# drnatebrown/col-bwt

Hardware: AMD Instinct MI355X
Metric: query bases/s (higher is better)
Workload: dtype int64

## Files before the change

### col-bwt_amd/__init__.py

```python
import ctypes as C
import os

import numpy as np

_HERE = os.path.dirname(os.path.abspath(__file__))
LIB_PATH = os.path.join(_HERE, "libcolbwt.so")
HEADER_PATH = os.path.join(os.path.dirname(_HERE), "include", "colbwt.h")

EXPORTS = (
    "colbwt_version", "colbwt_last_error", "colbwt_index_open", "colbwt_index_open_memory",
    "colbwt_index_open_layout", "colbwt_index_open_memory_layout",
    "colbwt_index_open_devices", "colbwt_index_open_memory_devices",
    "colbwt_index_close", "colbwt_index_info", "colbwt_query_batch", "colbwt_query_batch_u32",
    "colbwt_query_device", "colbwt_query_device_ordered", "colbwt_query_file", "colbwt_query_file_binary",
    "colbwt_binary_to_text", "colbwt_synth_index_bytes", "colbwt_synth_index", "colbwt_synth_index_thr", "colbwt_pml_pack_device", "colbwt_read_end_mask_device", "colbwt_pml_unpack_device",
    "colbwt_index_cid_dictionary", "colbwt_cid_code_bits", "colbwt_cid_pack_device", "colbwt_cid_unpack_device",
    "colbwt_synth_reads_device", "colbwt_build_col_pml", "colbwt_build_col_pml_arrays",
    "colbwt_col_split", "colbwt_col_split_arrays", "colbwt_col_split_error",
    "colbwt_rlbwt_build_text", "colbwt_rlbwt_build_files", "colbwt_rlbwt_get", "colbwt_rlbwt_free", "colbwt_rlbwt_error",
    "colbwt_count_batch", "colbwt_count_device", "colbwt_count_file",
    "colbwt_index_attach_locate", "colbwt_index_attach_locate_memory", "colbwt_locate_docs", "colbwt_locate_batch",
    "colbwt_locate_device", "colbwt_locate_file",
    "colbwt_rlbwt_build_text_locate", "colbwt_rlbwt_build_files_locate", "colbwt_rlbwt_write_locate",
    "colbwt_seeds_reduce_device", "colbwt_seeds_batch", "colbwt_seeds_file",
)

SEED_NONE = 0xFFFFFFFF
SEED_SUMMARY = np.dtype([(k, np.uint32) for k in ("n_seeds", "max_len", "cov", "resets", "n_col", "col_cov", "asc", "desc")])
LOCATE_NONE = (1 << 64) - 1


class ColbwtError(RuntimeError):
    def __init__(self, code, msg):
        super().__init__(f"colbwt error {code}: {msg}")
        self.code = code


class Info(C.Structure):
    _fields_ = [("bwt_r", C.c_uint64), ("n", C.c_uint64), ("r", C.c_uint64), ("sigma", C.c_uint32),
                ("device", C.c_uint32), ("device_bytes", C.c_uint64), ("layout", C.c_uint32),
                ("layout_shape", C.c_uint32), ("table_rows", C.c_uint64), ("n_devices", C.c_uint32),
                ("reserved_", C.c_uint32)]


class Stats(C.Structure):
    _fields_ = [("n_reads", C.c_uint64), ("n_bases", C.c_uint64), ("h2d_ms", C.c_double),
                ("kernel_ms", C.c_double), ("d2h_ms", C.c_double), ("algorithmic_bytes", C.c_uint64)]

    def as_dict(self):
        return {k: getattr(self, k) for k, _ in self._fields_}


_lib = None


def lib():
    global _lib
    if _lib is not None:
        return _lib
    if not os.path.exists(LIB_PATH):
        raise ColbwtError(-100, f"{LIB_PATH} not built: run __graft_entry__.build() "
                                "(the query path has no CPU fallback)")
    try:
        import torch
    except ImportError:
# ... 77 lines not shown
        else:
            _check(lib().colbwt_index_open_layout(os.fsencode(prefix_or_file), None, int(device), int(layout),
                                                  C.byref(h)))
        return cls(h)

    @classmethod
    def from_bytes(cls, image, device=0, layout=0, devices=None):
        arr = np.ascontiguousarray(np.frombuffer(image, dtype=np.uint8))
        h = C.c_void_p()
        if devices is not None:
            dv = (C.c_int * len(devices))(*[int(d) for d in devices])
            _check(lib().colbwt_index_open_memory_devices(arr.ctypes.data, arr.size, None, dv, len(devices), int(layout),
                                                          C.byref(h)))
        else:
            _check(lib().colbwt_index_open_memory_layout(arr.ctypes.data, arr.size, None, int(device), int(layout),
                                                         C.byref(h)))
        return cls(h)

    def info(self):
        out = Info()
        _check(lib().colbwt_index_info(self._h, C.byref(out)))
        return out

    def query_pml(self, pattern):
        p = np.frombuffer(bytes(pattern), dtype=np.uint8)
        off = np.array([0, p.size], dtype=np.uint64)
        pml, cid, _ = self.query_batch(p, off, wide=p.size > 65535)
        return pml.astype(np.uint64), cid.astype(np.uint64)

    def query_batch(self, bases, read_off, wide=False):
        bases = np.ascontiguousarray(bases, dtype=np.uint8)
        read_off = np.ascontiguousarray(read_off, dtype=np.uint64)
        n_reads = read_off.size - 1
        total = int(read_off[-1]) if n_reads >= 0 and read_off.size else 0
        pml = np.zeros(total, np.uint32 if wide else np.uint16)
        cid = np.zeros(total, np.uint8)
        st = Stats()
        fn = lib().colbwt_query_batch_u32 if wide else lib().colbwt_query_batch
        _check(fn(self._h, bases.ctypes.data, read_off.ctypes.data, max(n_reads, 0),
                  pml.ctypes.data, cid.ctypes.data, C.byref(st)))
        return pml, cid, st

    def query_device(self, d_bases, d_read_off, n_reads, n_bases, d_pml, d_cid, pml_bytes=2,
                     stream=0, timed=False, d_order=None):
        st = Stats()
        _check(lib().colbwt_query_device_ordered(self._h, d_bases, d_read_off, n_reads, n_bases, d_pml,
# ... 329 lines not shown
```

### col-bwt_amd/csrc/capi.hip

```cpp
#include <fcntl.h>
#include <hip/hip_runtime.h>
#include <stdlib.h>
#include <string.h>
#include <sys/mman.h>
#include <sys/stat.h>
#include <unistd.h>

#include <algorithm>
#include <atomic>
#include <chrono>
#include <condition_variable>
#include <deque>
#include <mutex>
#include <string>
#include <thread>
#include <vector>

#include "../../include/colbwt.h"
#include "bin_writer.h"
#include "count_query.h"
#include "fasta_parallel.h"
#include "fastx_reader.h"
#include "index.h"
#include "locate_query.h"
// ... 859 lines not shown
int colbwt_index_open_devices(const char *prefix_or_file, const colbwt_widths *widths, const int *devices, int n_devices,
                              int layout, colbwt_index **out) {
    if (!prefix_or_file || !out) return fail(COLBWT_ERR_ARG, "null argument");
    *out = nullptr;
    MappedFile mf;
    const int rc = map_index_file(prefix_or_file, mf);
    return rc != COLBWT_OK ? rc : colbwt_index_open_memory_devices(mf.data, mf.len, widths, devices, n_devices, layout, out);
}

void colbwt_index_close(colbwt_index *idx) { delete idx; }

int colbwt_index_info(const colbwt_index *idx, colbwt_info *out) {
    if (!idx || !out) return fail(COLBWT_ERR_ARG, "null argument");
    out->bwt_r = idx->ix.bwt_r();
    out->n = idx->ix.n();
    out->r = idx->ix.r();
    out->sigma = idx->ix.sigma();
    out->device = (uint32_t)idx->ix.device();
    out->device_bytes = idx->ix.device_bytes() + idx->loc.bytes();
    out->layout = (uint32_t)idx->ix.layout();
    out->layout_shape = idx->ix.line_rows() ? (idx->ix.table_fat().steps << 8) | kFatSlotSteps : 0;
    out->table_rows = idx->ix.table_rows();
    out->n_devices = 1 + (uint32_t)idx->more.size();
    out->reserved_ = 0;
    return COLBWT_OK;
}

int colbwt_query_batch(colbwt_index *idx, const uint8_t *bases, const uint64_t *read_off, uint64_t n_reads,
                       uint16_t *pml, uint8_t *cid, colbwt_stats *stats) {
    return query_batch_all<uint16_t>(idx, bases, read_off, n_reads, pml, cid, stats);
}

int colbwt_query_batch_u32(colbwt_index *idx, const uint8_t *bases, const uint64_t *read_off, uint64_t n_reads,
                           uint32_t *pml, uint8_t *cid, colbwt_stats *stats) {
    return query_batch_all<uint32_t>(idx, bases, read_off, n_reads, pml, cid, stats);
}

int colbwt_query_device(colbwt_index *idx, const uint8_t *d_bases, const uint64_t *d_read_off, uint64_t n_reads,
                        uint64_t n_bases, void *d_pml, int pml_bytes, uint8_t *d_cid, void *hip_stream,
                        colbwt_stats *stats) {
    return colbwt_query_device_ordered(idx, d_bases, d_read_off, n_reads, n_bases, d_pml, pml_bytes, d_cid, nullptr,
                                       hip_stream, stats);
}

int colbwt_query_device_ordered(colbwt_index *idx, const uint8_t *d_bases, const uint64_t *d_read_off,
                                uint64_t n_reads, uint64_t n_bases, void *d_pml, int pml_bytes, uint8_t *d_cid,
                                const uint32_t *d_order, void *hip_stream, colbwt_stats *stats) {
// ... 507 lines not shown
```

### col-bwt_amd/csrc/fat2_query.hip

```cpp
#include <hip/hip_runtime.h>
#include <stdint.h>

#include "device_layout.h"
#include "fat_cursor.h"
#include "fat_layout.h"
#include "lane_io.h"
#include "lane_out.h"
#include "query_kernels.h"

namespace colbwt {

namespace {

constexpr uint32_t kOffMis0 = 0xFFFFFFFCu;
constexpr uint32_t kOffMis1 = 0xFFFFFFFBu;

#ifdef COLBWT_COUNT_TRIPS
#define FAT2_STAT(k) (++stat[k])
#else
#define FAT2_STAT(k) ((void)0)
#endif

__device__ __forceinline__ uint32_t mis_slot(const uint8_t *top, uint32_t own, uint32_t c) {
    const uint32_t aidx = top[own], cidx = top[c];
// ... 21 lines not shown
    uint32_t *const claim = &s_claim;
    ReadCursor rc;
    bool done;
    rc.c_next = threadIdx.x;
    rc.request_chunk(plan, read_off);
    rc.commit();
    done = !rc.enter_chunk(plan, claim);

    OutRuns acc;
    uint32_t trip = 0;
    LaneWindow win;
    win.init(rc.off + rc.k - 1);
    uint4 (*const my_win)[64] = s_win[wave];

    uint32_t j = done ? 0u : T.r - 1;
    uint32_t o = kOffLastPos;
    uint32_t L = 0;
    const uint4 *const my_row = &s_stage[wave][p][g8];

#ifdef COLBWT_COUNT_TRIPS
    unsigned long long stat[8] = {0, 0, 0, 0, 0, 0, 0, 0};
#endif
    while (__any(!done)) {
        bool step_back = false;
        if (!done && rc.k == 0 && !rc.next_in_flight && (rc.r != rc.r_lo || rc.nc_ready)) {
            if (rc.r != rc.r_lo) {
                rc.r -= 1;
                rc.k = rc.off - rc.next_off;
                rc.off = rc.next_off;
                step_back = rc.r > rc.r_lo;
            } else if (kWide || acc.cnt == 0) {
                done = !rc.enter_chunk(plan, claim);
                if (!done) win.init(rc.off + rc.k - 1);
            }
            j = done ? 0u : T.r - 1;
            o = kOffLastPos;
            L = 0;
        }
        const bool live = !done && rc.k != 0;
        uint64_t &k = rc.k;
        const uint64_t g = rc.off + k - 1;

        s_jx[lane] = j;
        wave_sync();
        {
            const uint4 ja = *reinterpret_cast<const uint4 *>(&s_jx[g8]);
            const uint4 jb = *reinterpret_cast<const uint4 *>(&s_jx[g8 + 4]);
            const uint32_t jq[8] = {ja.x, ja.y, ja.z, ja.w, jb.x, jb.y, jb.z, jb.w};
            wave_sync();
#pragma unroll
            for (uint32_t q = 0; q < 8; ++q)
                __builtin_amdgcn_global_load_lds(T.lines + (uint64_t)jq[q] * kFatRowBytes + ((p ^ q) << 4), &s_stage[wave][q][0],
                                                 16, 0, 0);
        }
        if (live && win.avail(g) < (k < 8u ? (uint32_t)k : 8u)) win.request(my_win, bases, g);
        if (step_back) { rc.in_next = read_off[rc.r - 1]; rc.next_in_flight = true; }
        if (!done && rc.fetch_pending) rc.request_chunk(plan, read_off);
        lds_dma_landed();
        rc.commit();

        const uint32_t have = live ? win.avail(g) : 0u;
        uint32_t consumed = 0, l_new = 0, keep = 0xFFFFFFFFu, keep1 = 0xFFFFFFFFu;
        uint64_t ids = 0;
        if (!live || have == 0) FAT2_STAT(5);
        if (live && have != 0) {
            const uint64_t W = win.get8(my_win, lane, g);
            const uint32_t left = k < have ? (uint32_t)k : have;
            if (o == kOffMis0 || o == kOffMis1) {
                FAT2_STAT(2);
                const uint32_t h4 = !kDeep && o == kOffMis1 ? 4u : 0u;
                const uint4 e0 = my_row[(h4 + 0u) ^ p], e1 = my_row[(h4 + 1u) ^ p], e2 = my_row[(h4 + 2u) ^ p],
                            e3 = my_row[(h4 + 3u) ^ p];
                const uint32_t carry = L;
                const uint32_t t1 = (e0.y >> 16) & 0xFFu, d1 = e0.y >> 24, v1 = e3.z & 7u;
                uint32_t oc = 4;
                if (left >= 2) {
                    const uint32_t c2 = (uint32_t)(W >> 48) & 0xFFu;
                    const uint32_t s2 = mis_slot(s_top, t1, c2);
                    if (c2 == t1) oc = 0;
                    else if (s2 < kFatSlots && ((v1 >> s2) & 1u)) oc = 1 + s2;
                }
                if (oc < 4) {
                    const uint32_t J = oc == 0 ? e0.z : oc == 1 ? e0.w : oc == 2 ? e1.x : e1.y;
                    const uint32_t rho = oc == 0 ? e1.z : oc == 1 ? e1.w : oc == 2 ? e2.x : e2.y;
                    const uint32_t pw = oc < 2 ? e2.z : e2.w, P = (oc & 1u) ? pw >> 16 : pw & 0xFFFFu;
// ... 27 lines not shown
                        uint32_t sn = kFatSlots;
                        if (left > seen) {
                            const uint32_t cn = (uint32_t)(W >> (8u * (7u - seen))) & 0xFFu;
                            if (cn != nch) sn = mis_slot(s_top, nch, cn);
                        }
                        if (sn < kFatSlots && ((nv >> sn) & 1u)) {
                            const uint32_t e = nrho * kFatSlots + sn;
                            j = T.slot_line0 + (kDeep ? e : e >> 1);
                            o = kDeep ? kOffMis0 : kOffMis0 - (e & 1u);
                            L = ncd;
                        } else {
                            j = nJ;
                            o = nP;
                        }
                    }
                } else {
                    consumed = 1;
                    l_new = 0;
                    ids = (uint64_t)carry;
                    L = 0;
                    j = e0.x;
                    o = e0.y & 0xFFFFu;
                }
            } else {
                FAT2_STAT(0);
                const uint4 r0 = my_row[0 ^ p];
                const uint4 r1 = my_row[1 ^ p];
                const uint64_t CH = (uint64_t)r0.x | ((uint64_t)r0.y << 32);
                const uint64_t CID = (uint64_t)r0.z | ((uint64_t)r0.w << 32);
                const uint32_t len = r1.x & 0xFFFFu;
                uint32_t skip = 0;
                bool stay = false;
                if (o == kOffPred) { o = len - 1; skip = 1; }
                else if (o == kOffSucc) { o = 0; skip = 1; }
                else if (o >= len && j < T.r - 1) {
                    o -= len;
                    j += 1;
                    stay = true;
                    FAT2_STAT(1);
                } else {
                    o = o < len ? o : len - 1;
                }
                if (!stay) {
                    const uint64_t X = skip ? ((W >> 8) ^ CH) & 0x00FFFFFFFFFFFFFFull : W ^ CH;
                    const uint32_t run = matching_top_bytes(X);
                    const uint32_t cap = left + skip < (uint32_t)K ? left + skip : (uint32_t)K;
// ... 48 lines not shown
                        const uint32_t Oh = reinterpret_cast<const uint16_t *>(&my_row[((kFatO / 16) + (e >> 3)) ^ p])[e & 7u];
                        const uint64_t cuts = (uint64_t)r1.y | ((uint64_t)r1.z << 32);
                        const uint32_t cut = (uint32_t)(cuts >> (8 * e)) & 0xFFu, cut_a = cut & 0xFu, len_b = cut >> 4;
                        j = I;
                        if (cut_a != kSKCutNone && o >= cut_a) {
                            j += 1;
                            o -= cut_a;
                            if (len_b != kSKCutNone && o >= len_b) {
                                j += 1;
                                o -= len_b;
                            }
                        } else {
                            o += Oh;
                        }
                    }
                }
            }
            if constexpr (kWide) {
                for (uint32_t e = 0; e < consumed; ++e) {
                    pml[g - consumed + 1 + e] = (PmlT)((e < 2 ? keep : keep1) ? l_new - e : 0u);
                    cid[g - consumed + 1 + e] = (uint8_t)(ids >> (8 * e));
                }
            } else {
                acc.push_run(consumed, l_new, keep, keep1, (uint32_t)ids, (uint32_t)(ids >> 32));
            }
            k -= consumed;
        }
        wave_sync();
        if constexpr (!kWide) {
#ifdef COLBWT_ABL_NO_FLUSH
            if ((trip & (OutRuns::kPeriod - 1)) == OutRuns::kPeriod - 1) acc.cnt = acc.cnt > 90 ? 1 : 0;
#else
            if ((trip & (OutRuns::kPeriod - 1)) == OutRuns::kPeriod - 1)
                acc.flush_wave((uint16_t *)pml, cid, rc.off + rc.k, !done, rc.k == 0 && rc.r == rc.r_lo, &s_stage[wave][0][0], lane);
#endif
        }
        ++trip;
        wave_sync();
    }
#ifdef COLBWT_COUNT_TRIPS
    for (int q = 0; q < 8; ++q) atomicAdd(&g_fat_stats[q], stat[q]);
#endif
}

template <int K>
void launch_steps2(const FatTable &T, const uint8_t *d_bases, const uint64_t *d_read_off, uint64_t n_reads, uint64_t n_bases,
                   void *d_pml, int pml_bytes, uint8_t *d_cid, hipStream_t stream) {
// ... 31 lines not shown
```

### col-bwt_amd/csrc/fat_build.hip

```cpp
#include <hip/hip_runtime.h>
#include <stdint.h>

#include <functional>
#include <string>
#include <vector>

#include "../../include/colbwt.h"
#include "dev_mem.h"
#include "device_layout.h"
#include "fat_layout.h"
#include "jump_tables.h"
#include "lf_device.h"
#include "query_kernels.h"
#include "read_sampler.h"
#include "refine.h"

namespace colbwt {

namespace {

struct PlainLevel {
    const uint64_t *idx;
    const uint32_t *I;
    const uint16_t *O;
// ... 286 lines not shown
            w[kMisJ + o] = j;
            w[kMisRho + o] = rho[j];
            put_half(w, 4 * kMisP + 2 * o, (uint32_t)t);
            put_byte(w, 4 * kMisCh + o, m & 0xFFu);
            put_byte(w, 4 * kMisCid + o, m >> 8);
            w[kMisVal] |= (uint32_t)(sflags[j] & 7u) << (4 + 4 * o);
            if constexpr (kDeep) {
                plain_lf(P, j, t);
                const uint32_t m2 = P.meta[j];
                w[kMisDeep + kMisJ - 2 + o] = j;
                w[kMisDeep + kMisRho - 2 + o] = rho[j];
                put_half(w, 4 * (kMisDeep + kMisP - 2) + 2 * o, (uint32_t)t);
                put_byte(w, 4 * (kMisDeep + kMisCh - 2) + o, m2 & 0xFFu);
                put_byte(w, 4 * (kMisDeep + kMisCid - 2) + o, m2 >> 8);
                w[kMisDeep + kMisVal - 2] |= (uint32_t)(sflags[j] & 7u) << (4 * o);
            }
        }
    }
    uint4 *dst = reinterpret_cast<uint4 *>(entries + e * (kDwords * 4));
#pragma unroll
    for (uint32_t q = 0; q < kDwords / 4; ++q) dst[q] = make_uint4(w[4 * q], w[4 * q + 1], w[4 * q + 2], w[4 * q + 3]);
}

template <class Src>
int refine_plain(const Src &S, uint64_t src_rows, uint64_t n, PlainLevel &out, PlainBuffers &buf, std::string &err) {
    DevPtr first, park;
    uint64_t total = 0;
    {
        const int rc = count_and_scan(S, src_rows, first, total, err);
        if (rc != COLBWT_OK) return rc;
    }
    if (total > 0xFFFFFFFEull) {
        err = "line-row layout needs " + std::to_string(total) + " rows at one of its levels (> 2^32-2)";
        return COLBWT_ERR_NOMEM;
    }
    if (total * kFatRowBytes > dev_available_bytes()) {
        if (getenv("COLBWT_ALLOC_LOG"))
            fprintf(stderr, "[colbwt alloc] ? %llu rows x 128 bytes = %.2f GB against %.2f GB available\n", (unsigned long long)total,
                    total * 128e-9, dev_available_bytes() * 1e-9);
        err = "line-row layout: " + std::to_string(total) + " rows at a refinement level need more HBM than is available";
        return COLBWT_ERR_NOMEM;
    }
    const uint32_t r_new = (uint32_t)total;
    SK_TRY(buf.idx.alloc(((uint64_t)r_new + 2) * sizeof(uint64_t)));
    SK_TRY(buf.I.alloc(((uint64_t)r_new + 1) * sizeof(uint32_t)));
    SK_TRY(buf.O.alloc(((uint64_t)r_new + 1) * sizeof(uint16_t)));
// ... 123 lines not shown
            mismatch_lines = deep_bytes + kDeepReserve <= dev_available_bytes() ? 2 : 1;
        }
        const uint32_t entry_shift = mismatch_lines == 2 ? 7u : 6u;
        mis_lines = ((n_rho * kFatSlots << entry_shift) + kFatRowBytes - 1) / kFatRowBytes;
        if ((uint64_t)r + 1 + mis_lines > 0xFFFFFFFEull) {
            err = "line rows + mismatch lines need " + std::to_string((uint64_t)r + 1 + mis_lines) + " lines (> 2^32-2)";
            return COLBWT_ERR_NOMEM;
        }
        out.n_rho = (uint32_t)n_rho;
        out.slot_line0 = r + 1;
        out.entry_shift = entry_shift;
        SK_TRY(rho_first_buf.alloc((n_rho + 1) * sizeof(uint32_t)));
        SK_TRY(sflags_buf.alloc((uint64_t)r + 1));
        d_rho_first = rho_first_buf.as<uint32_t>();
        d_sflags = sflags_buf.as<uint8_t>();
        hipLaunchKernelGGL(rho_kernel, dim3(nblocks), dim3(256), 0, 0, d_org, r, d_rho, d_rho_first);
        SK_TRY(hipGetLastError());
        hipLaunchKernelGGL(fat_slot_flags_kernel, dim3(nblocks), dim3(256), 0, 0, cur, out, (const uint32_t *)d_rho,
                           (const uint32_t *)d_rho_first, d_sflags);
        SK_TRY(hipGetLastError());
        SK_TRY(hipStreamSynchronize(0));
        clock.lap("  origin rows, entry flags");
    }
    {
        PlainAllocScope whole;
        SK_TRY(buf.lines.alloc(((uint64_t)r + 1 + mis_lines) * kFatRowBytes));
    }
    clock.lap("  lines allocated");
    uint8_t *const d_lines = buf.lines.as<uint8_t>();
    SK_TRY(hipMemset(d_lines + (uint64_t)r * kFatRowBytes, 0, kFatRowBytes));
    if (mismatch_lines) {
        hipLaunchKernelGGL((fat_pack_kernel<K, true>), dim3(nblocks), dim3(256), 0, 0, cur, out, (const uint32_t *)d_rho,
                           (const uint8_t *)d_sflags, d_lines);
        SK_TRY(hipGetLastError());
        uint8_t *const d_entries = d_lines + ((uint64_t)r + 1) * kFatRowBytes;
        if (mis_lines) SK_TRY(hipMemset(d_entries + (mis_lines - 1) * kFatRowBytes, 0, kFatRowBytes));
        const uint64_t n_entries = (uint64_t)out.n_rho * kFatSlots;
        if (mismatch_lines == 2)
            hipLaunchKernelGGL(fat_mis_pack_kernel<true>, dim3((uint32_t)((n_entries + 255) / 256)), dim3(256), 0, 0, cur, out,
                               (const uint32_t *)d_rho, (const uint32_t *)d_rho_first, (const uint8_t *)d_sflags, d_entries);
        else
            hipLaunchKernelGGL(fat_mis_pack_kernel<false>, dim3((uint32_t)((n_entries + 255) / 256)), dim3(256), 0, 0, cur, out,
                               (const uint32_t *)d_rho, (const uint32_t *)d_rho_first, (const uint8_t *)d_sflags, d_entries);
    } else {
        hipLaunchKernelGGL((fat_pack_kernel<K, false>), dim3(nblocks), dim3(256), 0, 0, cur, out, (const uint32_t *)nullptr,
                           (const uint8_t *)nullptr, d_lines);
    }
    SK_TRY(hipGetLastError());
    SK_TRY(hipStreamSynchronize(0));
    out.lines = d_lines;
    clock.lap("  lines packed");
    buf.idx = std::move(cur_buf.idx);
    buf.thr = std::move(cur_buf.thr);
    cur_buf.release();
    clock.lap("  level arrays freed");
    return COLBWT_OK;
}

struct FatView {
    FatTable T;
    struct Row {
        uint32_t i1, o1_len, ch;
    };
    __device__ __forceinline__ uint64_t n() const { return T.n; }
    __device__ __forceinline__ uint32_t rows() const { return T.r; }
    __device__ __forceinline__ uint64_t idx(uint32_t j) const { return T.idx[j]; }
    __device__ __forceinline__ Row load(uint32_t j) const {
        const uint32_t *p = reinterpret_cast<const uint32_t *>(T.lines + (uint64_t)j * kFatRowBytes);
        Row w;
        w.i1 = p[kFatI / 4];
        w.o1_len = fat_half(p, kFatO) | (fat_half(p, kFatLen) << 16);
        w.ch = fat_byte(p, kFatCh + 7);
        return w;
    }
// ... 55 lines not shown
```

### col-bwt_amd/csrc/fat_cursor.h

```cpp
#pragma once
#include <hip/hip_runtime.h>
#include <stdint.h>
#include <stdlib.h>
#include <string.h>

#include <algorithm>

#include "device_layout.h"
#include "fat_layout.h"
#include "lane_io.h"
#include "query_kernels.h"

namespace colbwt {

namespace {

constexpr uint32_t kOffLastPos = 0xFFFFFFFFu;
constexpr uint32_t kOffPred = 0xFFFFFFFEu;
constexpr uint32_t kOffSucc = 0xFFFFFFFDu;
constexpr uint32_t kWaves = kQueryBlock / 64;

__device__ __forceinline__ bool fat_threshold_scan(const FatTable &T, uint32_t &j, uint32_t &o, uint32_t c, uint32_t cidx) {
    const uint64_t pos = T.idx[j] + o;
    uint64_t thr = T.n;
    uint32_t nj = j, no = o;
    bool moved = false;
    const uint32_t s = fat_succ_char(T, j, c, cidx);
    if (s != kNone) { thr = T.thr[s]; nj = s; no = kOffSucc; moved = true; }
    if (pos < thr) {
        const uint32_t q = fat_pred_char(T, j, c, cidx);
        if (q != kNone) { nj = q; no = kOffPred; moved = true; }
    }
    j = nj;
    o = no;
    return moved;
}

#ifdef COLBWT_COUNT_TRIPS
__device__ unsigned long long g_fat_stats[8];
__device__ unsigned long long g_fat_clocks[8];
#define FAT_STAT(k) (++stat[k])
#define FAT_CLOCK(k) do { const unsigned long long t_ = clock64(); clk[k] += t_ - t_prev; t_prev = t_; } while (0)
#else
#define FAT_STAT(k) ((void)0)
#define FAT_CLOCK(k) ((void)0)
#endif

__device__ __forceinline__ uint32_t matching_top_bytes(uint64_t x) {
    return x ? (uint32_t)__builtin_clzll(x) >> 3 : 8u;
}

struct ChunkPlan {
    uint64_t read_lo;
    uint64_t n_big, n_chunks;
    uint32_t big;
    __device__ __forceinline__ void init(uint64_t n_reads, uint32_t big_reads, uint32_t tail_permille) {
        read_lo = n_reads / gridDim.x * blockIdx.x + (n_reads % gridDim.x < blockIdx.x ? n_reads % gridDim.x : blockIdx.x);
        const uint64_t n = n_reads / gridDim.x + (blockIdx.x < n_reads % gridDim.x ? 1 : 0);
        uint64_t tail = n * tail_permille / 1000;
        tail = tail < 2 * kQueryBlock ? 2 * kQueryBlock : tail;
        tail = tail < n ? tail : n;
        big = big_reads;
        n_big = (n - tail) / big;
        n_chunks = n_big + (n - n_big * big);
    }
    __device__ __forceinline__ uint64_t first_read(uint64_t c) const {
        return read_lo + (c < n_big ? c * big : n_big * big + (c - n_big));
    }
    __device__ __forceinline__ uint64_t last_read(uint64_t c) const {
        return read_lo + (c < n_big ? (c + 1) * big - 1 : n_big * big + (c - n_big));
    }
};
// ... 75 lines not shown
```

### col-bwt_amd/csrc/fat_layout.h

```cpp
#pragma once
#include <hip/hip_runtime.h>
#include <stdint.h>

#include "device_layout.h"

namespace colbwt {

#define COLBWT_FAT_STEPS(X) X(4) X(5) X(6) X(7) X(8)

constexpr uint32_t kFatRowBytes = 128;
constexpr uint32_t kFatSlots = 3;
constexpr uint32_t kFatSlotSteps = 2;
constexpr uint32_t kFatOwnOther = 7;
constexpr uint32_t kFatCh = 0, kFatCid = 8, kFatLen = 16, kFatFlags = 18, kFatCut = 20, kFatI = 32, kFatO = 64,
                   kFatSlot0 = 80, kFatSlotBytes = 16;
constexpr uint32_t kFatSlotP = 8, kFatSlotCh2 = 12, kFatSlotCid2 = 13;
constexpr uint32_t kFatVal = 28, kFatRho = 80;
constexpr uint32_t kMisBytes = 64, kMisJ1 = 0, kMisP1 = 1, kMisJ = 2, kMisRho = 6, kMisP = 10, kMisCh = 12, kMisCid = 13, kMisVal = 14;
constexpr uint32_t kMisDeep = 16;

struct FatTable {
    const uint8_t *lines;
    const uint8_t *chr;
    const uint64_t *idx;
    const uint64_t *thr;
    const uint32_t *next_tbl;
    const uint32_t *prev_tbl;
    const uint8_t *cmap;
    uint64_t n;
    uint32_t r;
    uint32_t sigma;
    uint32_t nblk;
    uint32_t steps;
    uint32_t top4;
    uint32_t slot_line0;
    uint32_t n_rho;
    uint32_t entry_shift;
};

__device__ __forceinline__ uint32_t fat_byte(const uint32_t *w, uint32_t off) { return (w[off >> 2] >> (8 * (off & 3u))) & 0xFFu; }
__device__ __forceinline__ uint32_t fat_half(const uint32_t *w, uint32_t off) { return (w[off >> 2] >> (8 * (off & 2u))) & 0xFFFFu; }

__device__ __forceinline__ uint32_t fat_top_index(uint32_t top4, uint32_t c) {
    uint32_t x = 4;
    x = ((top4 >> 24) & 0xFFu) == c ? 3u : x;
    x = ((top4 >> 16) & 0xFFu) == c ? 2u : x;
    x = ((top4 >> 8) & 0xFFu) == c ? 1u : x;
    x = (top4 & 0xFFu) == c ? 0u : x;
    return x;
}

__device__ __forceinline__ uint32_t fat_succ_char(const FatTable &T, uint32_t i, uint32_t c, uint32_t cidx) {
    const uint32_t blk = i >> kBlockShift;
    const uint64_t lim = (((uint64_t)blk + 1) << kBlockShift);
    const uint64_t end = lim < T.r ? lim : T.r;
    for (uint64_t s = (uint64_t)i + 1; s < end; ++s)
        if (T.chr[s] == c) return (uint32_t)s;
    if (blk + 1 < T.nblk) return T.next_tbl[(uint64_t)(blk + 1) * T.sigma + cidx];
    return kNone;
}
// ... 13 lines not shown
```

### col-bwt_amd/csrc/fat_query.hip

```cpp
#include <hip/hip_runtime.h>
#include <stdint.h>

#include "device_layout.h"
#include "fat_cursor.h"
#include "fat_layout.h"
#include "lane_io.h"
#include "lane_out.h"
#include "query_kernels.h"

namespace colbwt {

namespace {

template <int K, typename PmlT>
__global__ __launch_bounds__(kQueryBlock)
void fat_query_kernel(FatTable T, const uint8_t *__restrict__ bases, const uint64_t *__restrict__ read_off,
                      uint64_t n_reads, uint32_t big_reads, uint32_t tail_permille,
                      PmlT *__restrict__ pml, uint8_t *__restrict__ cid) {
    constexpr bool kWide = sizeof(PmlT) == 4;
    __shared__ uint4 s_stage[kWaves][8][64];
    __shared__ uint4 s_win[kWaves][4][64];
    __shared__ uint32_t s_claim;
    const uint32_t wave = threadIdx.x >> 6, lane = threadIdx.x & 63u, g8 = lane & ~7u, p = lane & 7u;
    uint32_t *const s_jx = reinterpret_cast<uint32_t *>(&s_stage[wave][7][48]);
// ... 5 lines not shown
    ReadCursor rc;
    bool done;
    rc.c_next = threadIdx.x;
    rc.request_chunk(plan, read_off);
    rc.commit();
    done = !rc.enter_chunk(plan, claim);

    OutRuns acc;
    uint32_t trip = 0;
    LaneWindow win;
    win.init(rc.off + rc.k - 1);
    uint4 (*const my_win)[64] = s_win[wave];

    uint32_t j = done ? 0u : T.r - 1;
    uint32_t o = kOffLastPos;
    uint32_t L = 0;
    const uint4 *const my_row = &s_stage[wave][p][g8];

#ifdef COLBWT_COUNT_TRIPS
    unsigned long long stat[8] = {0, 0, 0, 0, 0, 0, 0, 0};
    unsigned long long clk[8] = {0, 0, 0, 0, 0, 0, 0, 0}, t_prev = clock64();
#endif
    while (__any(!done)) {
        bool step_back = false;
        if (!done && rc.k == 0 && !rc.next_in_flight && (rc.r != rc.r_lo || rc.nc_ready)) {
            if (rc.r != rc.r_lo) {
                rc.r -= 1;
                rc.k = rc.off - rc.next_off;
                rc.off = rc.next_off;
                step_back = rc.r > rc.r_lo;
            } else if (kWide || acc.cnt == 0) {
                FAT_STAT(6);
                done = !rc.enter_chunk(plan, claim);
                if (!done) win.init(rc.off + rc.k - 1);
            }
            j = done ? 0u : T.r - 1;
            o = kOffLastPos;
            L = 0;
        }
        FAT_CLOCK(4);
        const bool live = !done && rc.k != 0;
        uint64_t &k = rc.k;
        const uint64_t g = rc.off + k - 1;

        s_jx[lane] = j;
        wave_sync();
        {
            const uint4 ja = *reinterpret_cast<const uint4 *>(&s_jx[g8]);
            const uint4 jb = *reinterpret_cast<const uint4 *>(&s_jx[g8 + 4]);
            const uint32_t jq[8] = {ja.x, ja.y, ja.z, ja.w, jb.x, jb.y, jb.z, jb.w};
            wave_sync();
#pragma unroll
            for (uint32_t q = 0; q < 8; ++q)
                __builtin_amdgcn_global_load_lds(T.lines + (uint64_t)jq[q] * kFatRowBytes + ((p ^ q) << 4), &s_stage[wave][q][0],
                                                 16, 0, 0);
        }
        FAT_CLOCK(5);
        FAT_CLOCK(6);
        if (live && win.avail(g) < (k < 8u ? (uint32_t)k : 8u)) win.request(my_win, bases, g);
        if (step_back) { rc.in_next = read_off[rc.r - 1]; rc.next_in_flight = true; }
        if (!done && rc.fetch_pending) rc.request_chunk(plan, read_off);
        FAT_CLOCK(1);
        lds_dma_landed();
        rc.commit();
        FAT_CLOCK(2);

        const uint32_t have = live ? win.avail(g) : 0u;
        if (!live || have == 0) FAT_STAT(5);
        if (live && have != 0) {
            FAT_STAT(0);
            const uint4 r0 = my_row[0 ^ p];
            const uint4 r1 = my_row[1 ^ p];
            const uint64_t CH = (uint64_t)r0.x | ((uint64_t)r0.y << 32);
            const uint32_t len = r1.x & 0xFFFFu, flags = (r1.x >> 16) & 0xFFu;
            uint32_t skip = 0;
            bool stay = false;
            if (o == kOffPred) { o = len - 1; skip = 1; FAT_STAT(7); }
            else if (o == kOffSucc) { o = 0; skip = 1; FAT_STAT(7); }
            else if (o >= len && j < T.r - 1) {
                o -= len;
                j += 1;
                stay = true;
                FAT_STAT(1);
            } else {
                o = o < len ? o : len - 1;
            }
            if (!stay) {
                const uint64_t W = win.get8(my_win, lane, g);
                const uint64_t X = skip ? ((W >> 8) ^ CH) & 0x00FFFFFFFFFFFFFFull : W ^ CH;
                uint32_t steps = matching_top_bytes(X);
                const uint64_t left = k < have ? k : have;
                const uint32_t cap = left + skip < (uint64_t)K ? (uint32_t)left + skip : (uint32_t)K;
// ... 136 lines not shown
```

### col-bwt_amd/csrc/lane_out.h

```cpp
#pragma once
#include <hip/hip_runtime.h>
#include <stdint.h>

#include "lane_io.h"

#ifdef COLBWT_ABL_NO_STORES
#define COLBWT_ABL_IF if (ltop == 0xFFFFFFF1u)
#else
#define COLBWT_ABL_IF
#endif

namespace colbwt {

struct OutRuns {
    static constexpr uint32_t kBlock = 64;
    static constexpr uint32_t kPeriod = 4;
    static constexpr uint32_t kSlotQ = 6, kItemQ = 4;
    static constexpr uint32_t lds_q(uint32_t slots) { return slots * kSlotQ + 2 * slots * kItemQ; }

    uint32_t z0a = 0, z0b = 0, z0c = 0, z1a = 0, z1b = 0, z1c = 0;
    uint32_t ltop = 0;
    uint32_t c0 = 0, c1 = 0, c2 = 0, c3 = 0, c4 = 0, c5 = 0, c6 = 0, c7 = 0, c8 = 0, c9 = 0, c10 = 0, c11 = 0, c12 = 0, c13 = 0, c14 = 0, c15 = 0, c16 = 0, c17 = 0, c18 = 0, c19 = 0, c20 = 0, c21 = 0, c22 = 0, c23 = 0;
    uint32_t cnt = 0;

    __device__ __forceinline__ void push_run(uint32_t n, uint32_t l_new, uint32_t keep, uint32_t keep1, uint32_t ids_lo,
                                             uint32_t ids_hi) {
        const uint32_t in_run = (1u << n) - 1u;
        uint32_t p0 = l_new < n ? 1u << l_new : 0u;
        p0 |= (keep ? 0u : 3u) & in_run;
        p0 |= (keep1 ? 0u : 0xCu) & in_run;
        const uint32_t top = (1u << n) >> 1;
        const uint32_t p1 = (keep & keep1) != 0u && l_new == n ? top : 0u;
        z0c = (uint32_t)(((((uint64_t)z0c << 32) | z0b) << n) >> 32);
        z0b = (uint32_t)(((((uint64_t)z0b << 32) | z0a) << n) >> 32);
        z0a = (z0a << n) | p0;
        z1c = (uint32_t)(((((uint64_t)z1c << 32) | z1b) << n) >> 32);
        z1b = (uint32_t)(((((uint64_t)z1b << 32) | z1a) << n) >> 32);
        z1a = (z1a << n) | p1;
        const bool d4 = n & 8u, d2 = n & 4u;
        c23 = d4 ? c21 : c23;
        c22 = d4 ? c20 : c22;
        c21 = d4 ? c19 : c21;
        c20 = d4 ? c18 : c20;
        c19 = d4 ? c17 : c19;
        c18 = d4 ? c16 : c18;
        c17 = d4 ? c15 : c17;
        c16 = d4 ? c14 : c16;
        c15 = d4 ? c13 : c15;
        c14 = d4 ? c12 : c14;
        c13 = d4 ? c11 : c13;
        c12 = d4 ? c10 : c12;
        c11 = d4 ? c9 : c11;
        c10 = d4 ? c8 : c10;
        c9 = d4 ? c7 : c9;
        c8 = d4 ? c6 : c8;
// ... 239 lines not shown
```

### include/colbwt.h

```cpp
#ifndef COLBWT_H
#define COLBWT_H

#include <stddef.h>
#include <stdint.h>

#ifdef __cplusplus
extern "C" {
#endif

#define COLBWT_OK 0
#define COLBWT_ERR_ARG (-1)
#define COLBWT_ERR_IO (-2)
#define COLBWT_ERR_FORMAT (-3)
#define COLBWT_ERR_NO_DEVICE (-4)
#define COLBWT_ERR_HIP (-5)
#define COLBWT_ERR_NOMEM (-6)

typedef struct colbwt_index colbwt_index;

typedef struct colbwt_widths {
    uint32_t bwt_bytes;
    uint32_t run_bytes;
    uint32_t len_bytes;
    uint32_t id_bits;
} colbwt_widths;

typedef struct colbwt_info {
    uint64_t bwt_r;
    uint64_t n;
    uint64_t r;
    uint32_t sigma;
    uint32_t device;
    uint64_t device_bytes;
    uint32_t layout;
    uint32_t layout_shape;
    uint64_t table_rows;
    uint32_t n_devices;
    uint32_t reserved_;
} colbwt_info;

typedef struct colbwt_stats {
    uint64_t n_reads;
    uint64_t n_bases;
    double h2d_ms;
    double kernel_ms;
    double d2h_ms;
    uint64_t algorithmic_bytes;
} colbwt_stats;

const char *colbwt_version(void);
const char *colbwt_last_error(void);

int colbwt_index_open(const char *prefix_or_file, const colbwt_widths *widths, int device,
                      colbwt_index **out);
int colbwt_index_open_memory(const void *col_pml_bytes, uint64_t len, const colbwt_widths *widths,
                             int device, colbwt_index **out);
#define COLBWT_LAYOUT_AUTO 0
#define COLBWT_LAYOUT_ONE_STEP 1
#define COLBWT_LAYOUT_TWO_STEP 2
#define COLBWT_LAYOUT_THREE_STEP 3
#define COLBWT_LAYOUT_LINE_ROWS 4
// ... 143 lines not shown
```

Baseline: 146.9 billion.

## Add precomputed 8-base start table to skip initial backward steps per read

Builds a 65536-entry table at index build time that, for every 8-base suffix, stores the row, offset, match length, PML mask bits and colour ids reached after walking those 8 bases from the initial row. At the start of each read, both query kernels look up the last 8 bases and jump straight to that state, emitting 8 outputs in one step instead of iterating LF steps. This is meant to cut the per-read startup walk cost. In exchange it adds 2MB of device memory, a build-time kernel, a divergent lookup branch and extra register pressure in the hot loop.

```diff
diff --git a/col-bwt_amd/__init__.py b/col-bwt_amd/__init__.py
--- a/col-bwt_amd/__init__.py
+++ b/col-bwt_amd/__init__.py
@@ -40,7 +40,7 @@
     _fields_ = [("bwt_r", C.c_uint64), ("n", C.c_uint64), ("r", C.c_uint64), ("sigma", C.c_uint32),
                 ("device", C.c_uint32), ("device_bytes", C.c_uint64), ("layout", C.c_uint32),
                 ("layout_shape", C.c_uint32), ("table_rows", C.c_uint64), ("n_devices", C.c_uint32),
-                ("reserved_", C.c_uint32)]
+                ("start_entries", C.c_uint32)]
 
 
 class Stats(C.Structure):
@@ -164,6 +164,14 @@
         _check(lib().colbwt_index_info(self._h, C.byref(out)))
         return out
 
+    def debug_start_table(self):
+        fn = lib().colbwt_debug_start_table
+        fn.argtypes = [C.c_void_p, C.c_void_p, C.c_void_p]
+        entries = np.zeros(65536 * 32, np.uint8)
+        idx = np.zeros(int(self.info().table_rows) + 1, np.uint64)
+        _check(fn(self._h, entries.ctypes.data, idx.ctypes.data))
+        return entries, idx
+
     def query_pml(self, pattern):
         p = np.frombuffer(bytes(pattern), dtype=np.uint8)
         off = np.array([0, p.size], dtype=np.uint64)
diff --git a/col-bwt_amd/csrc/capi.hip b/col-bwt_amd/csrc/capi.hip
--- a/col-bwt_amd/csrc/capi.hip
+++ b/col-bwt_amd/csrc/capi.hip
@@ -905,7 +905,20 @@
     out->layout_shape = idx->ix.line_rows() ? (idx->ix.table_fat().steps << 8) | kFatSlotSteps : 0;
     out->table_rows = idx->ix.table_rows();
     out->n_devices = 1 + (uint32_t)idx->more.size();
-    out->reserved_ = 0;
+    out->start_entries = idx->ix.line_rows() && idx->ix.table_fat().start_line0 ? kStartEntries : 0;
+    return COLBWT_OK;
+}
+
+extern "C" int colbwt_debug_start_table(const colbwt_index *idx, void *entries_out, uint64_t *idx_out) {
+    if (!idx || !entries_out) return fail(COLBWT_ERR_ARG, "null argument");
+    if (!idx->ix.line_rows() || idx->ix.table_fat().start_line0 == 0) return fail(COLBWT_ERR_ARG, "the index has no start table");
+    const FatTable &T = idx->ix.table_fat();
+    if (hipSetDevice(idx->ix.device()) != hipSuccess) return fail(COLBWT_ERR_HIP, "hipSetDevice");
+    if (hipMemcpy(entries_out, T.lines + (uint64_t)T.start_line0 * kFatRowBytes, (uint64_t)kStartEntries * kStartBytes,
+                  hipMemcpyDeviceToHost) != hipSuccess)
+        return fail(COLBWT_ERR_HIP, "copying the start table");
+    if (idx_out && hipMemcpy(idx_out, T.idx, ((uint64_t)T.r + 1) * sizeof(uint64_t), hipMemcpyDeviceToHost) != hipSuccess)
+        return fail(COLBWT_ERR_HIP, "copying the row positions");
     return COLBWT_OK;
 }
 
diff --git a/col-bwt_amd/csrc/fat2_query.hip b/col-bwt_amd/csrc/fat2_query.hip
--- a/col-bwt_amd/csrc/fat2_query.hip
+++ b/col-bwt_amd/csrc/fat2_query.hip
@@ -67,7 +67,7 @@
     unsigned long long stat[8] = {0, 0, 0, 0, 0, 0, 0, 0};
 #endif
     while (__any(!done)) {
-        bool step_back = false;
+        bool step_back = false, fresh = false;
         if (!done && rc.k == 0 && !rc.next_in_flight && (rc.r != rc.r_lo || rc.nc_ready)) {
             if (rc.r != rc.r_lo) {
                 rc.r -= 1;
@@ -81,6 +81,19 @@
             j = done ? 0u : T.r - 1;
             o = kOffLastPos;
             L = 0;
+            fresh = !done;
+        }
+        if constexpr (!kWide) {
+            if (T.start_line0 != 0 && __any(fresh)) {
+                const uint64_t g0 = rc.off + rc.k - 1;
+                if (fresh && rc.k >= kStartBases && win.avail(g0) >= kStartBases) {
+                    const uint32_t e = start_entry_of(win.get8(my_win, lane, g0), [&](uint32_t c) { return (uint32_t)s_top[c]; });
+                    if (e != kNone) {
+                        j = T.start_line0 + (e >> 2);
+                        o = kOffStart + (e & 3u);
+                    }
+                }
+            }
         }
         const bool live = !done && rc.k != 0;
         uint64_t &k = rc.k;
@@ -106,6 +119,7 @@
 
         const uint32_t have = live ? win.avail(g) : 0u;
         uint32_t consumed = 0, l_new = 0, keep = 0xFFFFFFFFu, keep1 = 0xFFFFFFFFu;
+        uint32_t start_bits = 0;
         uint64_t ids = 0;
         if (!live || have == 0) FAT2_STAT(5);
         if (live && have != 0) {
@@ -179,6 +193,21 @@
                     j = e0.x;
                     o = e0.y & 0xFFFFu;
                 }
+            } else if (!kWide && o >= kOffStart && o < kOffStart + 4u) {
+                const uint32_t q2 = 2u * (o - kOffStart);
+                const uint4 s0 = my_row[q2 ^ p], s1 = my_row[(q2 + 1u) ^ p];
+                if (s0.y & kStartValid) {
+                    FAT2_STAT(7);
+                    consumed = kStartBases;
+                    start_bits = (s0.z & 0xFFFFu) | 0x10000u;
+                    ids = (uint64_t)s1.x | ((uint64_t)s1.y << 32);
+                    j = s0.x;
+                    o = s0.y & 0xFFFFu;
+                    L = (s0.y >> 16) & 0xFFu;
+                } else {
+                    j = T.r - 1;
+                    o = kOffLastPos;
+                }
             } else {
                 FAT2_STAT(0);
                 const uint4 r0 = my_row[0 ^ p];
@@ -273,7 +302,10 @@
                     cid[g - consumed + 1 + e] = (uint8_t)(ids >> (8 * e));
                 }
             } else {
-                acc.push_run(consumed, l_new, keep, keep1, (uint32_t)ids, (uint32_t)(ids >> 32));
+                uint32_t p0, p1;
+                OutRuns::run_masks(consumed, l_new, keep, keep1, p0, p1);
+                if (start_bits) { p0 = start_bits & 0xFFu; p1 = (start_bits >> 8) & 0xFFu; }
+                acc.push_masks(consumed, p0, p1, (uint32_t)ids, (uint32_t)(ids >> 32));
             }
             k -= consumed;
         }
diff --git a/col-bwt_amd/csrc/fat_build.hip b/col-bwt_amd/csrc/fat_build.hip
--- a/col-bwt_amd/csrc/fat_build.hip
+++ b/col-bwt_amd/csrc/fat_build.hip
@@ -1,5 +1,6 @@
 #include <hip/hip_runtime.h>
 #include <stdint.h>
+#include <stdlib.h>
 
 #include <functional>
 #include <string>
@@ -332,6 +333,50 @@
     for (uint32_t q = 0; q < kDwords / 4; ++q) dst[q] = make_uint4(w[4 * q], w[4 * q + 1], w[4 * q + 2], w[4 * q + 3]);
 }
 
+__global__ __launch_bounds__(256) void fat_start_kernel(PlainLevel P, FatTable T, uint8_t *__restrict__ entries) {
+    const uint32_t e = blockIdx.x * 256 + threadIdx.x;
+    if (e >= kStartEntries) return;
+    uint32_t j = P.r - 1;
+    uint64_t t = P.idx[P.r] - P.idx[P.r - 1] - 1;
+    uint32_t L = 0, z0 = 0, z1 = 0;
+    uint64_t ids = 0;
+    bool ok = true;
+    for (uint32_t s = 1; s <= kStartBases; ++s) {
+        const uint32_t code = (e >> (2 * (kStartBases - s))) & 3u, el = kStartBases - s;
+        const uint32_t c = (T.top4 >> (8 * code)) & 0xFFu;
+        ok = ok && code < T.sigma && fat_top_index(T.top4, c) == code;
+        const uint32_t meta = P.meta[j];
+        ids |= (uint64_t)(meta >> 8) << (8 * el);
+        if ((meta & 0xFFu) == c) {
+            ++L;
+            if (s == 1) z1 |= 1u << el;
+        } else {
+            L = 0;
+            z0 |= 1u << el;
+            const uint32_t cidx = T.cmap[c];
+            if (cidx != kAbsent) {
+                const uint64_t pos = P.idx[j] + t;
+                uint64_t thr = P.n;
+                uint32_t nj = j;
+                uint64_t nt = t;
+                const uint32_t sc = fat_succ_char(T, j, c, cidx);
+                if (sc != kNone) { thr = P.thr[sc]; nj = sc; nt = 0; }
+                if (pos < thr) {
+                    const uint32_t q = fat_pred_char(T, j, c, cidx);
+                    if (q != kNone) { nj = q; nt = P.idx[(uint64_t)q + 1] - P.idx[q] - 1; }
+                }
+                j = nj;
+                t = nt;
+            }
+        }
+        plain_lf(P, j, t);
+    }
+    ok = ok && t < P.idx[(uint64_t)j + 1] - P.idx[j] && t < 0xFFFFu;
+    uint4 *dst = reinterpret_cast<uint4 *>(entries + (uint64_t)e * kStartBytes);
+    dst[0] = ok ? make_uint4(j, (uint32_t)t | (L << 16) | kStartValid, z0 | (z1 << 8), 0u) : make_uint4(0u, 0u, 0u, 0u);
+    dst[1] = ok ? make_uint4((uint32_t)ids, (uint32_t)(ids >> 32), 0u, 0u) : make_uint4(0u, 0u, 0u, 0u);
+}
+
 template <class Src>
 int refine_plain(const Src &S, uint64_t src_rows, uint64_t n, PlainLevel &out, PlainBuffers &buf, std::string &err) {
     DevPtr first, park;
@@ -501,9 +546,12 @@
         SK_TRY(hipStreamSynchronize(0));
         clock.lap("  origin rows, entry flags");
     }
+    const char *const start_env = getenv("COLBWT_START_TABLE");
+    const bool start_table = !(start_env && atoi(start_env) == 0) && (uint64_t)r + 1 + mis_lines + kStartLines <= 0xFFFFFFFEull;
+    const uint64_t start_lines = start_table ? kStartLines : 0;
     {
         PlainAllocScope whole;
-        SK_TRY(buf.lines.alloc(((uint64_t)r + 1 + mis_lines) * kFatRowBytes));
+        SK_TRY(buf.lines.alloc(((uint64_t)r + 1 + mis_lines + start_lines) * kFatRowBytes));
     }
     clock.lap("  lines allocated");
     uint8_t *const d_lines = buf.lines.as<uint8_t>();
@@ -529,6 +577,14 @@
     SK_TRY(hipStreamSynchronize(0));
     out.lines = d_lines;
     clock.lap("  lines packed");
+    if (start_table) {
+        hipLaunchKernelGGL(fat_start_kernel, dim3(kStartEntries / 256), dim3(256), 0, 0, cur, out,
+                           d_lines + ((uint64_t)r + 1 + mis_lines) * kFatRowBytes);
+        SK_TRY(hipGetLastError());
+        SK_TRY(hipStreamSynchronize(0));
+        out.start_line0 = (uint32_t)((uint64_t)r + 1 + mis_lines);
+        clock.lap("  start table");
+    }
     buf.idx = std::move(cur_buf.idx);
     buf.thr = std::move(cur_buf.thr);
     cur_buf.release();
diff --git a/col-bwt_amd/csrc/fat_cursor.h b/col-bwt_amd/csrc/fat_cursor.h
--- a/col-bwt_amd/csrc/fat_cursor.h
+++ b/col-bwt_amd/csrc/fat_cursor.h
@@ -18,6 +18,7 @@
 constexpr uint32_t kOffLastPos = 0xFFFFFFFFu;
 constexpr uint32_t kOffPred = 0xFFFFFFFEu;
 constexpr uint32_t kOffSucc = 0xFFFFFFFDu;
+constexpr uint32_t kOffStart = 0xFFFFFFF4u;
 constexpr uint32_t kWaves = kQueryBlock / 64;
 
 __device__ __forceinline__ bool fat_threshold_scan(const FatTable &T, uint32_t &j, uint32_t &o, uint32_t c, uint32_t cidx) {
@@ -48,6 +49,18 @@
 
 __device__ __forceinline__ uint32_t matching_top_bytes(uint64_t x) {
     return x ? (uint32_t)__builtin_clzll(x) >> 3 : 8u;
+}
+
+template <class Top>
+__device__ __forceinline__ uint32_t start_entry_of(uint64_t W, Top top) {
+    uint32_t e = 0, any = 0;
+#pragma unroll
+    for (uint32_t i = 0; i < kStartBases; ++i) {
+        const uint32_t x = top((uint32_t)(W >> (8 * i)) & 0xFFu);
+        any |= x;
+        e |= (x & 3u) << (2 * i);
+    }
+    return any & 4u ? kNone : e;
 }
 
 struct ChunkPlan {
diff --git a/col-bwt_amd/csrc/fat_layout.h b/col-bwt_amd/csrc/fat_layout.h
--- a/col-bwt_amd/csrc/fat_layout.h
+++ b/col-bwt_amd/csrc/fat_layout.h
@@ -18,6 +18,10 @@
 constexpr uint32_t kFatVal = 28, kFatRho = 80;
 constexpr uint32_t kMisBytes = 64, kMisJ1 = 0, kMisP1 = 1, kMisJ = 2, kMisRho = 6, kMisP = 10, kMisCh = 12, kMisCid = 13, kMisVal = 14;
 constexpr uint32_t kMisDeep = 16;
+constexpr uint32_t kStartBases = 8, kStartEntries = 1u << (2 * kStartBases), kStartBytes = 32;
+constexpr uint32_t kStartLines = kStartEntries * kStartBytes / kFatRowBytes;
+constexpr uint32_t kStartJ = 0, kStartOL = 1, kStartBits = 2, kStartIds = 4;
+constexpr uint32_t kStartValid = 0x80000000u;
 
 struct FatTable {
     const uint8_t *lines;
@@ -36,6 +40,7 @@
     uint32_t slot_line0;
     uint32_t n_rho;
     uint32_t entry_shift;
+    uint32_t start_line0;
 };
 
 __device__ __forceinline__ uint32_t fat_byte(const uint32_t *w, uint32_t off) { return (w[off >> 2] >> (8 * (off & 3u))) & 0xFFu; }
diff --git a/col-bwt_amd/csrc/fat_query.hip b/col-bwt_amd/csrc/fat_query.hip
--- a/col-bwt_amd/csrc/fat_query.hip
+++ b/col-bwt_amd/csrc/fat_query.hip
@@ -51,7 +51,7 @@
     unsigned long long clk[8] = {0, 0, 0, 0, 0, 0, 0, 0}, t_prev = clock64();
 #endif
     while (__any(!done)) {
-        bool step_back = false;
+        bool step_back = false, fresh = false;
         if (!done && rc.k == 0 && !rc.next_in_flight && (rc.r != rc.r_lo || rc.nc_ready)) {
             if (rc.r != rc.r_lo) {
                 rc.r -= 1;
@@ -66,6 +66,19 @@
             j = done ? 0u : T.r - 1;
             o = kOffLastPos;
             L = 0;
+            fresh = !done;
+        }
+        if constexpr (!kWide) {
+            if (T.start_line0 != 0 && __any(fresh)) {
+                const uint64_t g0 = rc.off + rc.k - 1;
+                if (fresh && rc.k >= kStartBases && win.avail(g0) >= kStartBases) {
+                    const uint32_t e = start_entry_of(win.get8(my_win, lane, g0), [&](uint32_t c) { return fat_top_index(T.top4, c); });
+                    if (e != kNone) {
+                        j = T.start_line0 + (e >> 2);
+                        o = kOffStart + (e & 3u);
+                    }
+                }
+            }
         }
         FAT_CLOCK(4);
         const bool live = !done && rc.k != 0;
@@ -95,8 +108,24 @@
         FAT_CLOCK(2);
 
         const uint32_t have = live ? win.avail(g) : 0u;
+        const bool start_trip = !kWide && live && o >= kOffStart && o < kOffStart + 4u;
         if (!live || have == 0) FAT_STAT(5);
-        if (live && have != 0) {
+        if (start_trip) {
+            if constexpr (!kWide) {
+                const uint32_t q2 = 2u * (o - kOffStart);
+                const uint4 s0 = my_row[q2 ^ p], s1 = my_row[(q2 + 1u) ^ p];
+                if (s0.y & kStartValid) {
+                    acc.push_masks(kStartBases, s0.z & 0xFFu, (s0.z >> 8) & 0xFFu, s1.x, s1.y);
+                    k -= kStartBases;
+                    j = s0.x;
+                    o = s0.y & 0xFFFFu;
+                    L = (s0.y >> 16) & 0xFFu;
+                } else {
+                    j = T.r - 1;
+                    o = kOffLastPos;
+                }
+            }
+        } else if (live && have != 0) {
             FAT_STAT(0);
             const uint4 r0 = my_row[0 ^ p];
             const uint4 r1 = my_row[1 ^ p];
diff --git a/col-bwt_amd/csrc/lane_out.h b/col-bwt_amd/csrc/lane_out.h
--- a/col-bwt_amd/csrc/lane_out.h
+++ b/col-bwt_amd/csrc/lane_out.h
@@ -23,14 +23,22 @@
     uint32_t c0 = 0, c1 = 0, c2 = 0, c3 = 0, c4 = 0, c5 = 0, c6 = 0, c7 = 0, c8 = 0, c9 = 0, c10 = 0, c11 = 0, c12 = 0, c13 = 0, c14 = 0, c15 = 0, c16 = 0, c17 = 0, c18 = 0, c19 = 0, c20 = 0, c21 = 0, c22 = 0, c23 = 0;
     uint32_t cnt = 0;
 
-    __device__ __forceinline__ void push_run(uint32_t n, uint32_t l_new, uint32_t keep, uint32_t keep1, uint32_t ids_lo,
-                                             uint32_t ids_hi) {
+    static __device__ __forceinline__ void run_masks(uint32_t n, uint32_t l_new, uint32_t keep, uint32_t keep1, uint32_t &p0,
+                                                     uint32_t &p1) {
         const uint32_t in_run = (1u << n) - 1u;
-        uint32_t p0 = l_new < n ? 1u << l_new : 0u;
+        p0 = l_new < n ? 1u << l_new : 0u;
         p0 |= (keep ? 0u : 3u) & in_run;
         p0 |= (keep1 ? 0u : 0xCu) & in_run;
         const uint32_t top = (1u << n) >> 1;
-        const uint32_t p1 = (keep & keep1) != 0u && l_new == n ? top : 0u;
+        p1 = (keep & keep1) != 0u && l_new == n ? top : 0u;
+    }
+    __device__ __forceinline__ void push_run(uint32_t n, uint32_t l_new, uint32_t keep, uint32_t keep1, uint32_t ids_lo,
+                                             uint32_t ids_hi) {
+        uint32_t p0, p1;
+        run_masks(n, l_new, keep, keep1, p0, p1);
+        push_masks(n, p0, p1, ids_lo, ids_hi);
+    }
+    __device__ __forceinline__ void push_masks(uint32_t n, uint32_t p0, uint32_t p1, uint32_t ids_lo, uint32_t ids_hi) {
         z0c = (uint32_t)(((((uint64_t)z0c << 32) | z0b) << n) >> 32);
         z0b = (uint32_t)(((((uint64_t)z0b << 32) | z0a) << n) >> 32);
         z0a = (z0a << n) | p0;
diff --git a/include/colbwt.h b/include/colbwt.h
--- a/include/colbwt.h
+++ b/include/colbwt.h
@@ -36,7 +36,7 @@
     uint32_t layout_shape;
     uint64_t table_rows;
     uint32_t n_devices;
-    uint32_t reserved_;
+    uint32_t start_entries;
 } colbwt_info;
 
 typedef struct colbwt_stats {
```

New measurement: 135.9 billion. -7.5%, worse.
